# winlaic/ZipVoice

Measured on AMD Instinct MI355X. Metric: generated mel-frames/s (whole job) + RTF, ZipVoice 123M N_steps=16 batch=32/GPU, higher is better.
Workload: dtype bf16; 1 GPU; C2: ZipVoice 123M, N_steps=16, batch=32/GPU x (3 s prompt + 10 s generated; T=1219 frames), CFG g=1.0 (64 decoder rows per GPU), t_shift=0.5; model=zipvoice (zipvoice_base.json, synthetic seeded weights), global_batch=32, seq_len=1219, parallelism=dp1

## Files before the change

include/zipvoice_hip.h:

```cpp
#ifndef ZIPVOICE_HIP_H
#define ZIPVOICE_HIP_H

#include <stdint.h>

#ifdef __cplusplus
extern "C" {
#endif

typedef struct zv_engine* zv_handle;

enum zv_variant { ZV_ZIPVOICE = 0, ZV_DISTILL = 1, ZV_DIALOG = 2, ZV_DIALOG_STEREO = 3 };
enum zv_precision { ZV_FP32 = 0, ZV_BF16 = 1, ZV_MIXED = 2, ZV_FP8 = 3 };

#define ZV_MAX_STACKS 8

typedef struct {
  int variant;
  int precision;
  int feat_dim;
  int num_stacks;
  int downsampling_factor[ZV_MAX_STACKS];
  int num_layers[ZV_MAX_STACKS];
  int cnn_module_kernel[ZV_MAX_STACKS];
  int fm_decoder_dim, fm_decoder_feedforward_dim, fm_decoder_num_heads;
  int text_encoder_num_layers, text_encoder_feedforward_dim, text_encoder_cnn_module_kernel;
  int text_encoder_num_heads, text_encoder_dim;
  int time_embed_dim, text_embed_dim;
  int query_head_dim, value_head_dim, pos_head_dim, pos_dim;
  int vocab_size, pad_id, spk_a_id, spk_b_id;
} zv_config;

const char* zv_last_error(void);
const char* zv_version(void);

zv_handle zv_create(const zv_config* cfg);
void zv_destroy(zv_handle h);

int zv_set_weight(zv_handle h, const char* name, const float* host_data, int64_t numel);
int zv_finalize(zv_handle h);
int zv_reserve(zv_handle h, int max_batch, int max_frames);
int64_t zv_device_bytes(zv_handle h);

enum zv_padding { ZV_PAD_BATCH = 0, ZV_PAD_ROW = 1 };
int zv_set_padding(zv_handle h, int mode);
int zv_get_padding(zv_handle h);

int zv_profile(int enable);
int zv_profile_report(char* buf, int buflen);

int64_t zv_host_block_count(void);

int zv_attn_fallbacks(zv_handle h, int reset, int64_t* host_counts);

int zv_attn2_check(int kernel, int form, int B, int L, int H, int nv, const float* qkp, const float* P,
                   const uint8_t* key_pad, const float* v, const float* y, int force_exact, float* out,
                   int64_t* counts);

int zv_bench_gemm(int M, int N, int K, int variant, int iters, int out_mode, float* ms_out);

int zv_bench_fused_linear(int form, int M, int N, int K, int rpb, int iters, float* ms_out);

int zv_gemm_selftest(int M, int N, int K, int variant, int mode, float* maxdiff, float* maxref);

enum zv_linear_form {
  ZV_LIN_PLAIN = 0,
  ZV_LIN_PLAIN_F32 = 1,
  ZV_LIN_RESID = 2,
  ZV_LIN_RESID_BYP = 3,
  ZV_LIN_RESID_RV = 4,
  ZV_LIN_RESID_RV_COPY = 5,
  ZV_LIN_TRANS = 6,
  ZV_LIN_NA = 7,
  ZV_LIN_GLU = 8,
  ZV_LIN_GLU_DW = 9
};
typedef struct {
  int M, N, K, split, form, act;
  int rows_per_group;
  int rpb;
  int guard;
  const float* A; const float* W; const float* bias;
  const float* resid;
  const float* orig;
  const float* byp;
  const float* rowvec;
  const uint8_t* rowmask;
  const float* dw_w;
  const float* dw_b;
  int dw_ks, dw_L;
  float* C; int64_t ldc;
  uint16_t* Ch; uint16_t* Cl; int64_t ldch;
  uint16_t* Cth; uint16_t* Ctl; int64_t ldct;
  int launch[8];
  int num_cus;
} zv_linear_check_args;
int zv_linear_check(zv_linear_check_args* a);

typedef struct {
  int M, H, form, rows_per_group, part_slots, guard;
  float log_scale;
  const float* x; const float* W1; const float* b1; const float* W2; const float* b2;
  const float* resid;
  const float* rowvec;
  const float* orig;
  const float* byp;
  const float* nb;
  float* C; int64_t ldc;
  uint16_t* Ch; uint16_t* Cl; uint16_t* C2h; uint16_t* C2l; int64_t ldch;
  int launch[8];
// ... 323 lines not shown
```

zipvoice_amd/csrc/zv_checks.inc:

```
#pragma once

namespace {

struct ChkDev {
  std::vector<void*> ptrs;
  void* raw(size_t bytes) {
    void* p = nullptr;
    ZV_CHECK(ZV_BLOCKING(hipMalloc(&p, bytes + 256)));
    ptrs.push_back(p);
    return p;
  }
  template <typename T> T* make(size_t n) { return reinterpret_cast<T*>(raw(n * sizeof(T))); }
  template <typename T> T* zero(size_t n) {
    T* d = make<T>(n);
    ZV_CHECK(ZV_BLOCKING(hipMemset(d, 0, n * sizeof(T))));
    return d;
  }
  template <typename T> T* up(const T* host, size_t n) {
    T* d = make<T>(n);
    ZV_CHECK(ZV_BLOCKING(hipMemcpy(d, host, n * sizeof(T), hipMemcpyHostToDevice)));
    return d;
  }
  template <typename T> void down(T* host, const T* dev, size_t n) {
    ZV_CHECK(ZV_BLOCKING(hipMemcpy(host, dev, n * sizeof(T), hipMemcpyDeviceToHost)));
// ... 198 lines not shown
      p.Ch = reinterpret_cast<bf16*>(R) + (size_t)k * M * N;
      p.ldch = N;
    }
    if (mode == 2) {
      ZV_CHECK(hipMemcpyAsync(outs[k], R, mn * 4, hipMemcpyDeviceToDevice, s));
      p.resid = outs[k];
    }
    if (k == 0) launch_gemm<128, 128, 2, 2, 1, EPI_STD, 2, 2>(p, 1, s, "ref", true, 0);
    else if (variant == 70) launch_gemm<128, 128, 2, 2, 1, EPI_STD, 2, 2, GEMM_BK, 0, 0, 1>(p, 1, s, "t", true, -1);
    else if (variant == 71) launch_gemm<128, 128, 2, 2, 1, EPI_STD, 2, 2, GEMM_BK, 0, 0, 2>(p, 1, s, "t", true, -1);
    else launch_gemm<128, 128, 2, 2, 1, EPI_STD, 2, 2, GEMM_BK, 0, 0, 3>(p, 1, s, "t", true, -1);
  }
  if (bf16_out)
    for (int k = 0; k < 2; ++k)
      hipLaunchKernelGGL(zv_bf16_to_f32_kernel, dim3(1024), dim3(256), 0, s,
                         reinterpret_cast<bf16*>(R) + (size_t)k * M * N, outs[k], (long)M * N);
  ZV_CHECK(hipMemsetAsync(res, 0, 8, s));
  hipLaunchKernelGGL(zv_maxdiff_kernel, dim3(1024), dim3(256), 0, s, outs[1], outs[0], (long)M * N, res);
  float h[2];
  dev.down(h, res, 2);
  *maxdiff = h[0]; *maxref = h[1];
  ZV_API_END
}

int zv_attn_plan(int split, int sa_plo, int tpm, int L, int nv_na, int64_t* lds_sa, int64_t* lds_na,
                 int64_t* lds_stats, int* fits) {
  ZV_API_BEGIN
  ZV_REQUIRE((split == 1 || split == 3) && L > 0 && nv_na > 0 && sa_plo >= -1 && sa_plo <= 1 &&
                 tpm >= 0 && tpm <= 3 && (split == 1 || (sa_plo < 0 && tpm == 0)) && lds_sa && lds_na &&
                 lds_stats && fits,
             "bad arguments");
  if (tpm == 3) {
    *lds_sa = (int64_t)(sa3_qpw(L) ? sa3_plan_lds(L) : sa2_qpw(L) == 3 ? sa2_lds_bytes<3>(L) : sa2_lds_bytes<2>(L));
    *lds_na = (int64_t)(nv_na <= 128 ? na2_lds_bytes<1, 8>(L) : nv_na <= 256 ? na2_lds_bytes<2, 8>(L) : na2_lds_bytes<3, 8>(L));
    *lds_stats = 0;
    *fits = fused_attn2_fits(L, nv_na);
    return 0;
  }
  *lds_sa = (int64_t)(sa_plo < 0 ? sa_lds_bytes(L) : (sa_plo ? sa_tp_lds_bytes<1>(L) : sa_tp_lds_bytes<0>(L)));
  *lds_na = (int64_t)(split == 1 ? na_lds_bytes_for<1>(L, nv_na, tpm) : na_lds_bytes_for<3>(L, nv_na, tpm));
  *lds_stats = (int64_t)pos_mask_bytes(L, 64, true);
  *fits = split == 1 ? fused_attn_fits<1>(L, nv_na, sa_plo, tpm) : fused_attn_fits<3>(L, nv_na, sa_plo, tpm);
  ZV_API_END
}

int zv_attn2_check(int kernel, int form, int B, int L, int H, int nv, const float* qkp, const float* P,
                   const uint8_t* key_pad, const float* v, const float* y, int force_exact, float* out,
                   int64_t* counts) {
  ZV_API_BEGIN
  ZV_REQUIRE((kernel == 0 || kernel == 1) && B > 0 && L > 0 && H > 0 && qkp && P && v && out &&
                 (kernel == 0 ? (nv > 0 && nv <= 12) : (nv > 0 && nv <= 384 && y)),
             "zv_attn2_check: bad arguments");
  ZV_REQUIRE(kernel != 0 || (form >= 0 && form <= 5), "zv_attn2_check: SelfAttention form 0..5");
  ZV_REQUIRE(kernel != 1 || (form >= 0 && form <= 2), "zv_attn2_check: NonlinAttention form 0..2");
  const long ldq = 2L * H * ATT_QD + H * ATT_PD, M = (long)B * L, Lpad = round_up(L, 64);
  const long vrows = kernel == 0 ? 16L * H : nv;
  std::vector<bf16> hq((size_t)M * ldq), hv((size_t)B * vrows * Lpad, (bf16)0.f);
  for (size_t i = 0; i < hq.size(); ++i) hq[i] = (bf16)qkp[i];
  for (int b = 0; b < B; ++b)
    for (long r = 0; r < vrows; ++r) {
      const int h = kernel == 0 ? (int)(r / 16) : 0, d = kernel == 0 ? (int)(r % 16) : (int)r;
      for (int j = 0; j < L; ++j) {
        float x = 0.f;
        if (kernel == 1) x = v[((long)b * L + j) * nv + d];
        else if (d < nv) x = v[((long)b * L + j) * H * nv + (long)h * nv + d];
        else if (d == 12) x = 1.f;
        hv[((size_t)b * vrows + r) * Lpad + j] = (bf16)x;
      }
    }
  std::vector<bf16> hy;
  if (kernel == 1) {
    hy.resize((size_t)M * nv);
    for (size_t i = 0; i < hy.size(); ++i) hy[i] = (bf16)y[i];
  }
  const long ocols = kernel == 0 ? (long)H * nv : nv, ldo = round_up(ocols, 8);
  ChkDev dev;
  bf16* dout = dev.zero<bf16>((size_t)M * ldo);
  unsigned* dcnt = dev.zero<unsigned>(4);
  FlashParams f{};
  f.qh = dev.up(hq.data(), hq.size()); f.ldq = ldq;
  f.P = dev.up(P, (size_t)(2 * L - 1) * H * ATT_PD);
  f.key_pad = key_pad ? dev.up(key_pad, (size_t)M) : nullptr;
  f.B = B; f.L = L; f.H = H;
  f.vh = dev.up(hv.data(), hv.size()); f.ldv = Lpad; f.sv_b = vrows * Lpad; f.nv = nv;
  f.oh = dout; f.ldo = ldo;
  f.force_exact = force_exact; f.fallback = dcnt;
  hipStream_t s = nullptr;
  if (kernel == 0) {
    f.vrows_per_head = 16; f.ocol_per_head = nv;
    launch_attn_sa_b2(f, form ? form : sa_b2_form(L), s);
  } else {
    f.vrows_per_head = 0; f.ocol_per_head = 0;
    f.mulh = dev.up(hy.data(), hy.size()); f.ldmul = nv;
    launch_attn_na_b2(f, nv, form ? form : na_b2_form(L), s);
  }
  ZV_CHECK(ZV_BLOCKING(hipDeviceSynchronize()));
  std::vector<bf16> ho((size_t)M * ldo);
  dev.down(ho.data(), dout, ho.size());
  for (long m = 0; m < M; ++m)
    for (long c = 0; c < ocols; ++c) out[m * ocols + c] = (float)ho[m * ldo + c];
  if (counts) {
    unsigned c[4];
    dev.down(c, dcnt, 4);
    for (int i = 0; i < 3; ++i) counts[i] = c[i];
  }
  ZV_API_END
}

int zv_mx8_quantize(const float* x, int rows, int K, uint8_t* q, uint8_t* s) {
  ZV_API_BEGIN
  ZV_REQUIRE(x && q && s && rows >= 0 && K > 0, "bad arguments");
  mx8_quantize_host(x, K, rows, K, q, round_up(K, MX8_KSTEP), s);
  ZV_API_END
}

int zv_mx8_gemm_check(int M, int N, int K, const float* A, const float* W, float* C, uint8_t* Aq,
                      uint8_t* As) {
  ZV_API_BEGIN
  ZV_REQUIRE(A && W && C && M > 0 && N > 0 && K > 0 && K % MX8_KSTEP == 0 && N % 8 == 0,
             "zv_mx8_gemm_check: K a multiple of 128, N of 8");
  hipStream_t s = nullptr;
  const long Np = round_up(N, 128);
  std::vector<bf16> ah((size_t)M * K);
  for (size_t i = 0; i < ah.size(); ++i) ah[i] = (bf16)A[i];
  std::vector<float> wp((size_t)Np * K, 0.f);
  memcpy(wp.data(), W, (size_t)N * K * 4);
  std::vector<uint8_t> wq((size_t)Np * K), ws((size_t)Np * K / MX8_BLOCK);
  mx8_quantize_host(wp.data(), K, (int)Np, K, wq.data(), K, ws.data());
  ChkDev dev;
  uint8_t* dAq = dev.make<uint8_t>((size_t)M * K);
  uint8_t* dAs = dev.make<uint8_t>((size_t)M * K / MX8_BLOCK);
  const uint8_t* dWq = dev.up(wq.data(), wq.size());
  const uint8_t* dWs = dev.up(ws.data(), ws.size());
  float* dC = dev.zero<float>((size_t)M * N);
  Act a16;
  a16.h = dev.up(ah.data(), ah.size()); a16.ld = K;
  a16.q = dAq; a16.qs = dAs; a16.ldq = K;
  LinearPolicy().pack8(a16, M, K, s);
  GemmParams p{};
  p.M = M; p.N = N; p.K = K; p.nz2 = 1; p.Brows = (int)Np;
  p.Ah = reinterpret_cast<const bf16*>(dAq); p.lda = K; p.As = dAs; p.ldas = K / MX8_BLOCK;
  p.Bh = reinterpret_cast<const bf16*>(dWq); p.ldb = K; p.Bs = dWs; p.ldbs = K / MX8_BLOCK;
  p.bias = dev.zero<float>((size_t)N); p.C = dC; p.ldc = N; p.resid = dC; p.rows_per_group = 1; p.rpb = 1;
  launch_gemm<128, 128, 2, 2, 8, EPI_STD, 2, 2, MX8_KSTEP, 0, 0, 1>(p, 1, s, "mx8_check", true, -1);
  ZV_CHECK(ZV_BLOCKING(hipDeviceSynchronize()));
  dev.down(C, dC, (size_t)M * N);
  if (Aq) dev.down(Aq, dAq, (size_t)M * K);
  if (As) dev.down(As, dAs, (size_t)M * K / MX8_BLOCK);
  ZV_API_END
}

int zv_linear_check(zv_linear_check_args* a) {
  ZV_API_BEGIN
  ZV_REQUIRE(a && a->M > 0 && a->N > 0 && a->K > 0 && a->A && a->W && a->bias && a->guard >= 0 &&
                 (a->split == 1 || a->split == 2 || a->split == 3) && a->form >= ZV_LIN_PLAIN &&
                 a->form <= ZV_LIN_GLU_DW,
             "zv_linear_check: bad arguments");
  const int M = a->M, N = a->N, K = a->K, form = a->form, G = a->guard;
// ... 1107 lines not shown
```

zipvoice_amd/csrc/zv_engine.hip:

```cpp
#include <math.h>
#include <stdlib.h>
#include <string.h>

#include <algorithm>
#include <map>
#include <memory>
#include <mutex>
#include <string>
#include <exception>
#include <functional>
#include <tuple>
#include <vector>


#include "zv_common.h"
#include "zv_gemm.inc"
#include "zv_gemm256.inc"
#include "zv_ffn.inc"
#include "zv_attn.inc"
#include "zv_elem.inc"
#include "zv_session.inc"
#include "zv_flash.inc"
#include "zv_flash2.inc"
#include "zv_weights.inc"
// ... 131 lines not shown
  StreamSet set;
  set.dev = dev;
  for (int i = 0; i < ZV_STREAM_SET; ++i)
    ZV_CHECK(ZV_BLOCKING(hipStreamCreateWithFlags(&set.s[i], hipStreamNonBlocking)));
  return set;
}
static void release_stream_set(const StreamSet& set) {
  if (set.dev < 0) return;
  for (hipStream_t st : set.s)
    if (st) (void)ZV_BLOCKING(hipStreamSynchronize(st));
  std::lock_guard<std::mutex> lock(g_stream_pool_mu);
  stream_pool_free().push_back(set);
}

}

struct zv_engine;
struct zv_session {
  zv_engine* eng = nullptr;
  int slots = 0, maxT = 0;
  DBuf x, tc, sc, pad;
  float *dx = nullptr, *dtc = nullptr, *dsc = nullptr;
  uint8_t* dpad = nullptr;
  std::vector<SchedRow> rows;
  std::vector<std::vector<float>> ts;
  std::vector<int> lens, done;
  int64_t ticks = 0, dec_rows = 0, dec_row_frames = 0, last_T = 0;
  ~zv_session();
};

struct zv_engine : LinearPolicy {
  zv_config cfg;
  WeightStore store;
  ZipformerW dec, txt;
  float* embed_table = nullptr;
  float* spk_table = nullptr;
  float* temb_freqs = nullptr;
  Workspace ws_dec, ws_txt;
  static constexpr int MAX_SPLIT = 4;
  Workspace ws_split[MAX_SPLIT - 1];
  int split_streams = 3;
  long split_min_rows = 0;
  hipStream_t split_stream[MAX_SPLIT - 1] = {};
  hipEvent_t split_fork = nullptr, split_join[MAX_SPLIT - 1] = {};

  bool materialize_attn = false;
  int ffn_fused = 3;
  long ffn_min_rows = 15000;
  int fp8_fuse = 7;
  int sa_tp = 1;
  bool mixed_sa = true;
  bool attn_b2 = false, attn_b2_dec = false;
  int attn2_exact = 0;
  int glu_dw = 1;
  unsigned* attn_fallback = nullptr;
  int padding = ZV_PAD_BATCH;

  explicit zv_engine(const zv_config& c) : cfg(c) {
    auto envi = [](const char* k, int d) { const char* v = getenv(k); return v ? atoi(v) : d; };
    materialize_attn = envi("ZV_ATTN_MATERIALIZE", 0) == 1;
    graph_mode = envi("ZV_GRAPH", 2);
    sa_tp = envi("ZV_SA_TP", 1);
    fp8_fuse = envi("ZV_FP8_FUSE", 7);
    ffn_fused = envi("ZV_FFN", 3);
    ffn_min_rows = envi("ZV_FFN_MIN_ROWS", 15000);
    ffn_persist = envi("ZV_FFN_PERSIST", 1);
    split_streams = envi("ZV_SPLIT_STREAMS", 3);
    split_min_rows = envi("ZV_SPLIT_MIN_ROWS", 8192);
    mixed_sa = envi("ZV_MIXED_SA", 1) != 0;
    attn_b2 = envi("ZV_ATTN2", 1) != 0 && (cfg.precision == ZV_BF16 || cfg.precision == ZV_FP8);
    attn_b2_dec = attn_b2 || (envi("ZV_ATTN2", 1) != 0 && cfg.precision == ZV_MIXED);
    attn2_exact = envi("ZV_ATTN2_EXACT", 0) != 0;
    glu_dw = envi("ZV_GLU_DW", 1);
  }
  struct GraphKey {
    int B, T, N, has_pad;
    float g, t0, t1, shift;
    int cfg_mode;
    int padding;
    unsigned long gen;
    bool operator<(const GraphKey& o) const {
      return std::tie(B, T, N, has_pad, g, t0, t1, shift, cfg_mode, padding, gen) <
             std::tie(o.B, o.T, o.N, o.has_pad, o.g, o.t0, o.t1, o.shift, o.cfg_mode, o.padding, o.gen);
    }
  };
  static constexpr size_t MAX_GRAPHS = 8, MAX_SEEN = 256;
  struct GraphEntry { hipGraphExec_t exec; unsigned long last_use; };
  std::map<GraphKey, GraphEntry> graphs;
  std::map<GraphKey, int> graph_seen;
  unsigned long graph_clock = 0;
  hipStream_t gstream = nullptr;
  hipEvent_t gev_in = nullptr, gev_out = nullptr;
  DBuf gx, gtc, gsc, gpad, ggrows;
  int graph_mode = 2;

  int ffn_persist = 1;
  void attach_ffn_scratch(FfnParams& q, Workspace& ws) {
    if (!ffn_persist) return;
    const int cus = zv_num_cus();
    q.part = ws.ffn_part.get<float>((size_t)cus * FFN_PART_FLOATS);
    unsigned* fl = ws.ffn_flag.get<unsigned>((size_t)cus + 64);
    q.flag = fl;
    q.part_slots = cus;
  }
  void ffn_site(FfnParams q, Workspace& ws, hipStream_t s, const char* tag) {
    attach_ffn_scratch(q, ws);
    launch_ffn(q, s, tag);
  }

  void check_dev_err() {
    volatile unsigned* e = zv_dev_err_host();
    if (*e == 0) return;
    ZV_CHECK(ZV_BLOCKING(hipDeviceSynchronize()));
    auto clear = [](Workspace& w) {
      if (w.ffn_flag.p) ZV_CHECK(ZV_BLOCKING(hipMemset(w.ffn_flag.p, 0, w.ffn_flag.bytes)));
    };
    clear(ws_dec); clear(ws_txt);
    for (Workspace& w : ws_split) clear(w);
    ZV_CHECK(ZV_BLOCKING(hipDeviceSynchronize()));
    *e = 0;
    throw std::runtime_error("fused FeedForward: a C item waited more than 2 s for its producer's tiles; "
                             "the outputs of the calls since the previous one are invalid (schedule flags reset)");
  }

  void drop_graphs() {
// ... 274 lines not shown
                    false, attn_b2);
    embed_table = store.upload_key("embed.weight", (size_t)cfg.vocab_size * cfg.text_embed_dim);
    if (dialog()) spk_table = store.upload_key("spk_embed.weight", (size_t)2 * F);
    const int half = cfg.time_embed_dim / 2;
    std::vector<float> fr(half);
    for (int k = 0; k < half; ++k)
      fr[k] = expf((float)(-log(10000.0)) * (float)k / (float)half);
    temb_freqs = store.dalloc<float>(half);
    ZV_CHECK(ZV_BLOCKING(hipMemcpy(temb_freqs, fr.data(), half * sizeof(float), hipMemcpyHostToDevice)));
    attn_fallback = store.dalloc<unsigned>(4);
    ZV_CHECK(ZV_BLOCKING(hipMemset(attn_fallback, 0, 4 * sizeof(unsigned))));
    size_t expected = count_expected();
    if (expected != store.staged.size())
      throw std::invalid_argument("state dict has " + std::to_string(store.staged.size()) +
                                  " tensors, config expects " + std::to_string(expected) +
                                  " (unexpected keys present)");
    store.staged.clear();
    store.derived.clear();
    store.ready = true;
  }

  size_t count_expected() const {
    auto zf = [&](const ZipformerW& Z) {
      size_t n = 4 * Z.in_proj.size();
      for (const auto& S : Z.stacks) {
        if (S.ds != 1) n += 2;
        if (Z.temb_dim > 0) n += 2;
        n += S.layers.size() * 43;
      }
      if (Z.has_time) n += 4;
      if (Z.has_guid) n += 1;
      return n;
    };
    return zf(dec) + zf(txt) + 1 + (dialog() ? 1 : 0);
  }

  void small_linear(const Linear& L, const float* in, int ldin, int M, float* out, int ldout,
                    int pre, const float* add, hipStream_t s) {
    launch_small_linear(in, ldin, L.w32, L.K, L.b, add, out, ldout, M, L.N, L.K, pre, -1, s);
  }

  bool fp8_mode() const { return cfg.precision == ZV_FP8; }

  template <int SPLIT, int TPM>
  static void attn_na_v1(const FlashParams& f, int hid, hipStream_t s) {
    constexpr int QTILES = SPLIT == 3 ? 4 : 8;
    if (hid <= 128) launch_attn_na<SPLIT, 1, QTILES, TPM>(f, s);
    else if (hid <= 256) launch_attn_na<SPLIT, 2, QTILES, TPM>(f, s);
    else launch_attn_na<SPLIT, 3, QTILES, TPM>(f, s);
  }
  template <int SPLIT>
  void attn_na(const FlashParams& f, int hid, bool a2, bool tp_na, hipStream_t s) {
    if constexpr (SPLIT == 1) {
      if (a2) return launch_attn_na_b2(f, hid, na_b2_form(f.L), s);
      if (tp_na) return attn_na_v1<1, 1>(f, hid, s);
    }
    attn_na_v1<SPLIT, 0>(f, hid, s);
  }
  template <int SPLIT>
  void attn_sa(const FlashParams& f, bool a2, hipStream_t s) {
    if constexpr (SPLIT == 1) {
      if (a2) return launch_attn_sa_b2(f, sa_b2_form(f.L), s);
      if (sa_tp) {
        if (sa_tp == 3) launch_attn_sa_tp<0, 1>(f, s);
        else launch_attn_sa_tp<0>(f, s);
        return;
      }
    }
    launch_attn_sa<SPLIT>(f, s);
  }

  template <int SPLIT>
  void layer(const Pass& pass, const ZipformerW& Z, const LayerW& W, Workspace& ws, float* src,
             Act src_a, float* cur, Act cur_a, int B, int L, const uint8_t* pad, const float* posP,
             const float* temb, bool has_next, hipStream_t s, bool fresh8 = false) {
    const bool split = SPLIT == 3;
    const long M = (long)B * L;
    const long Mtot = pass.batch_rows > 0 ? pass.batch_rows * (long)L : M;
    const int D = Z.dim, H = Z.heads;
    const long Lpad = round_up(L, 64);
    const char* tag_att = split ? "gemm_attn_fp32" : "gemm_attn_bf16";
    const int qkpN = W.attn_in.N;
    Act qkp = ws.qkp.get(M, qkpN, split);
    {
      Out o; o.act = qkp;
      if (SPLIT == 1 && pass.io_split) attn_in_wsplit(W.attn_in, src_a, M, o, s);
      else linear<SPLIT>(W.attn_in, src_a, M, o, s);
    }
    const bool tp_na = SPLIT == 1 && sa_tp;
    const int sa_plo = (SPLIT == 1 && sa_tp) ? 0 : -1;
    const bool a2 = SPLIT == 1 && Z.b2;
    const bool materialize = materialize_attn || (a2 ? !fused_attn2_fits(L, W.na_in.N / 3)
                                                     : !fused_attn_fits<SPLIT>(L, W.na_in.N / 3, sa_plo, tp_na ? 1 : 0));
    Act Wt;
    FlashParams fp{};
    if (materialize) {
      Wt = ws.W.get((long)H * M, Lpad, split);
      AttnParams ap{qkp.h, qkp.l, qkpN, posP, pad, Wt.h, Wt.l, Lpad, B, L, H, a2 ? 1 : 0};
      launch_attn_softmax<SPLIT>(ap, s);
    } else {
      fp.qh = qkp.h; fp.ql = qkp.l; fp.ldq = qkpN; fp.P = posP; fp.key_pad = pad;
      fp.B = B; fp.L = L; fp.H = H;
      fp.force_exact = attn2_exact; fp.fallback = attn_fallback;
      if (!a2) {
        fp.stats = ws.stats.get<float2>((size_t)M);
        if constexpr (SPLIT == 1)
          if (tp_na) launch_attn_stats<1, 1>(fp, s);
// ... 1347 lines not shown
```

zipvoice_amd/csrc/zv_flash2.inc:

```
#pragma once
#include "zv_flash.inc"

constexpr float FA2_MASKED = -1000.f * 1.4426950408889634f;
constexpr float FA2_DEN_LO = 8.673617379884035e-19f;
constexpr float FA2_DEN_HI = 1.2676506002282294e30f;
constexpr int SA2_KS = 64;
constexpr bool FA2_OFS = std::is_same<bf16, _Float16>::value;
#ifndef ZV_FA2_DIAG
#define ZV_FA2_DIAG 1
#endif

template <int KS>
__device__ __forceinline__ void stage_bias2(const FlashParams& p, int b, float* Mb, uint8_t* Fs, int tid,
                                            int nt) {
  const int L = p.L, nks = (L + KS - 1) / KS, NM = nks * KS;
  for (int k = tid; k < nks; k += nt) Fs[k] = 0;
  __syncthreads();
  const uint8_t* kp = p.key_pad ? p.key_pad + (long)b * L : nullptr;
  for (int t = tid; t < NM; t += nt) {
    const int m = t >= L ? 2 : (kp ? kp[t] : 0);
    Mb[t] = m == 0 ? 0.f : (m == 1 ? FA2_MASKED : -INFINITY);
    if (m) Fs[t / KS] = 1;
  }
  __syncthreads();
// ... 519 lines not shown
      c = ZV_MFMA_16x16x32(ldk(ks * FA_KB), qf, c, 0, 0, 0);
      c = ZV_MFMA_16x16x32(PP[jb + tbl], pb[0], c, 0, 0, 0);
      c = ZV_MFMA_16x16x32(PP[jb + tbl - 8], pb[1], c, 0, 0, 0);
      mx = fmaxf(mx, fmaxf(fmaxf(c[0], c[1]), fmaxf(c[2], c[3])));
    }
    half_sums(mx, true);
    const float rowmax = ceilf(fmaxf(Qs[sq * 16 + c16], Qs[QT + sq * 16 + c16]));
    cofs = f32x4{0.f, 0.f, 0.f, 0.f};
    __syncthreads();
    key_loop(rowmax);
    half_sums(psum, false);
  }

#pragma unroll
  for (int q = 0; q < 4; ++q) {
    const int ql = (aq0 + q) * 16 + c16;
    const int qo = qt0 + ql;
    if (qo >= L) continue;
    const float rden = 1.f / (Qs[ql] + Qs[QT + ql]);
    const long orow = (long)b * L + qo;
#pragma unroll
    for (int t = 0; t < DTW; ++t) {
      const int d0 = (ad0 + t) * 16 + g * 4;
      if (d0 >= nv) continue;
      float v[4] = {acc[q][t][0], acc[q][t][1], acc[q][t][2], acc[q][t][3]};
      float y[4];
      load_split4(p.mulh, (const bf16*)nullptr, orow * p.ldmul + d0, y);
#pragma unroll
      for (int e = 0; e < 4; ++e) v[e] *= y[e] * rden;
      store_split4(p.oh, nullptr, orow * p.ldo + d0, v);
    }
  }
}

inline int na2_qtiles(int L) { return L <= 900 ? 4 : 8; }

template <int DTW, int QTILES = 8>
static void launch_attn_na2(const FlashParams& p, hipStream_t s) {
  const size_t lds = na2_lds_bytes<DTW, QTILES>(p.L);
  ZV_REQUIRE(lds <= 160 * 1024, "sequence too long for the fused attention kernel");
  ZV_REQUIRE(p.nv <= 8 * DTW * 16 && !p.ol && p.ldq % 8 == 0, "NonlinAttention v2 operands");
  static unsigned long long attr = 0;
  if (!((attr >> zv_cur_device()) & 1)) {
    ZV_CHECK(hipFuncSetAttribute((const void*)zv_attn_na2_kernel<DTW, QTILES>,
                                 hipFuncAttributeMaxDynamicSharedMemorySize, 160 * 1024));
    attr |= 1ull << zv_cur_device();
  }
  const long nblk = (long)cdiv(p.L, 16 * QTILES) * p.B;
  ZvProfScope prof("attn_na_bf16", (72.0 + 2.0 * p.nv) * p.B * (double)p.L * p.L, 0.0, s);
  hipLaunchKernelGGL((zv_attn_na2_kernel<DTW, QTILES>), dim3((unsigned)nblk), dim3(128 * QTILES), lds, s, p);
  ZV_LAUNCH_CHECK();
}

constexpr int SA3_SLOT = 6144;
template <int QPW>
__host__ __device__ inline size_t sa3_lds_bytes(int L) {
  const int nks = (L + SA2_KS - 1) / SA2_KS;
  return (size_t)3 * SA3_SLOT + (size_t)(L + 64 * QPW + SA2_KS) * 16 + (size_t)nks * SA2_KS * 4 + round_up(nks, 16);
}

inline int sa3_qpw(int L) {
  if (L <= 400) return 0;
  if (L >= 1500 && sa3_lds_bytes<3>(L) <= 80 * 1024) return 3;
  if (L >= 1000 && L < 1500 && sa3_lds_bytes<4>(L) <= 80 * 1024) return 4;
  return sa3_lds_bytes<2>(L) <= 80 * 1024 ? 2 : 0;
}
inline int sa2_qpw(int L) { return L > 400 && sa2_lds_bytes<3>(L) <= 160 * 1024 ? 3 : 2; }
inline size_t sa3_plan_lds(int L) {
  const int q = sa3_qpw(L);
  return q == 4 ? sa3_lds_bytes<4>(L) : q == 3 ? sa3_lds_bytes<3>(L) : q == 2 ? sa3_lds_bytes<2>(L) : 0;
}

template <int QPW, int MINW = 2>
__global__ __launch_bounds__(256, MINW) void zv_attn_sa3_kernel(FlashParams p) {
  constexpr int QT = 64 * QPW, KS = SA2_KS, NU = QPW + 3;
  extern __shared__ __attribute__((aligned(16))) unsigned char fsm[];
  const int L = p.L;
  const int nks = (L + KS - 1) / KS;
  const int NT = L + QT + KS;
  unsigned char* ring = fsm;
  bf16x8* PP = reinterpret_cast<bf16x8*>(fsm + 3 * SA3_SLOT);
  float* Mb = reinterpret_cast<float*>(PP + NT);
  uint8_t* Fs = reinterpret_cast<uint8_t*>(Mb + nks * KS);

  const int nqb = (L + QT - 1) / QT;
  const int lb = fa2_xcd_block(blockIdx.x, gridDim.x);
  const int qt0 = (lb % nqb) * QT, h = (lb / nqb) % p.H, b = lb / nqb / p.H;
  const int tid = threadIdx.x, lane = tid & 63;
  const int wave = __builtin_amdgcn_readfirstlane(tid >> 6);
  const int g = lane >> 4, c16 = lane & 15;
  const long qbase = (long)b * L * p.ldq;

  const int ldqb = (int)p.ldq * 2, ldvb = (int)p.ldv * 2;
  const char* kbase = reinterpret_cast<const char*>(p.qh + qbase + p.H * ATT_QD + h * ATT_QD);
  const char* vbase = reinterpret_cast<const char*>(p.vh + (long)b * p.sv_b + (long)h * 16 * p.ldv);
  const unsigned k_lane = (unsigned)(c16 * ldqb + g * 16);
  const int vrow = 8 * (wave & 1) + (lane >> 3);
  const unsigned v_lane = (unsigned)(vrow * ldvb + (((lane & 7) ^ ((vrow >> 1) & 7)) * 16));
  auto issue = [&](int ks) {
    unsigned char* slot = ring + (ks % 3) * SA3_SLOT;
    const int j0 = ks * KS, jk = j0 + 16 * wave;
    if (jk + 16 <= L) {
      glds16s(kbase + (long)jk * ldqb, k_lane, slot + wave * 1024);
    } else {
      const unsigned kc = (unsigned)(min(jk + c16, L - 1) * ldqb + g * 16);
      glds16s(kbase, kc, slot + wave * 1024);
// ... 188 lines not shown
  }

#pragma unroll
  for (int qq = 0; qq < QPW; ++qq) {
    const int d0 = g * 4;
    if (qi[qq] >= L || d0 >= p.nv) continue;
    const float rden = 1.f / den[qq];
    float v[4] = {acc[qq][0] * rden, acc[qq][1] * rden, acc[qq][2] * rden, acc[qq][3] * rden};
    const long o = ((long)b * L + qi[qq]) * p.ldo + (long)h * p.ocol_per_head + d0;
    if (d0 + 3 < p.nv) {
      store_split4(p.oh, p.ol, o, v);
      if (p.oh2) store_split4(p.oh2, nullptr, o, v);
    } else {
      for (int e = 0; d0 + e < p.nv; ++e) {
        split_store(p.oh, p.ol, o + e, v[e]);
        if (p.oh2) split_store(p.oh2, nullptr, o + e, v[e]);
      }
    }
  }
}

template <int QPW = 2, int MINW = 2>
static void launch_attn_sa3(const FlashParams& p, hipStream_t s) {
  const size_t lds = sa3_lds_bytes<QPW>(p.L);
  ZV_REQUIRE(lds <= 160 * 1024, "sequence too long for the fused attention kernel");
  ZV_REQUIRE(p.nv <= 12 && p.vrows_per_head == 16 && p.ldq % 8 == 0 && p.ldv % 64 == 0,
             "SelfAttention v3: 16-row value heads (row 12 = ones), V^T rows padded to 64 keys");
  static unsigned long long attr = 0;
  if (!((attr >> zv_cur_device()) & 1)) {
    ZV_CHECK(hipFuncSetAttribute((const void*)zv_attn_sa3_kernel<QPW, MINW>,
                                 hipFuncAttributeMaxDynamicSharedMemorySize, 160 * 1024));
    attr |= 1ull << zv_cur_device();
  }
  const long nblk = (long)cdiv(p.L, 64 * QPW) * p.H * p.B;
  ZV_REQUIRE(nblk < (1L << 31), "SelfAttention v3 grid");
  ZvProfScope prof("attn_sa_bf16", (72.0 + 2.0 * p.nv) * p.H * p.B * (double)p.L * p.L, 0.0, s);
  hipLaunchKernelGGL((zv_attn_sa3_kernel<QPW, MINW>), dim3((unsigned)nblk), dim3(256), lds, s, p);
  ZV_LAUNCH_CHECK();
}

inline int sa_b2_form(int L) {
  const int q3 = sa3_qpw(L);
  return q3 ? q3 + 1 : sa2_qpw(L) == 3 ? 2 : 1;
}
static void launch_attn_sa_b2(const FlashParams& f, int form, hipStream_t s) {
  switch (form) {
    case 1: launch_attn_sa2<2>(f, s); break;
    case 2: launch_attn_sa2<3, 1>(f, s); break;
    case 3: launch_attn_sa3<2>(f, s); break;
    case 4: launch_attn_sa3<3>(f, s); break;
    default: launch_attn_sa3<4>(f, s); break;
  }
}
inline int na_b2_form(int L) { return na2_qtiles(L) == 4 ? 1 : 2; }
static void launch_attn_na_b2(const FlashParams& f, int hid, int form, hipStream_t s) {
  if (hid <= 128) { if (form == 1) launch_attn_na2<1, 4>(f, s); else launch_attn_na2<1>(f, s); }
  else if (hid <= 256) { if (form == 1) launch_attn_na2<2, 4>(f, s); else launch_attn_na2<2>(f, s); }
  else if (form == 1) launch_attn_na2<3, 4>(f, s);
  else launch_attn_na2<3>(f, s);
}

static bool fused_attn2_fits(int L, int nv_na) {
  const size_t lim = 160 * 1024;
  const size_t na = nv_na <= 128 ? na2_lds_bytes<1, 8>(L) : nv_na <= 256 ? na2_lds_bytes<2, 8>(L) : na2_lds_bytes<3, 8>(L);
  return sa2_lds_bytes<2>(L) <= lim && na <= lim;
}
```

zipvoice_amd/engine.py:

```python
from __future__ import annotations

import ctypes
import os
from typing import Dict, Optional

import numpy as np
import torch

from .config import ModelConfig
from .weights import check_state_dict

LIB_NAME = "libzipvoice_hip.so"
LIB_PATH = os.path.join(os.path.dirname(os.path.abspath(__file__)), LIB_NAME)
LIB_F16_PATH = os.path.join(os.path.dirname(os.path.abspath(__file__)), "libzipvoice_hip_f16.so")
MAX_STACKS = 8
VARIANT_ID = {"zipvoice": 0, "zipvoice_distill": 1, "zipvoice_dialog": 2,
              "zipvoice_dialog_stereo": 3}
PRECISION_ID = {"fp32": 0, "bf16": 1}
MODES = {"fp32": ("bf16", 0), "bf16": ("bf16", 1), "fp16": ("f16", 2),
         "fp16_plain": ("f16", 1), "bf16_mixed": ("bf16", 2), "fp8": ("bf16", 3)}


class ZvConfig(ctypes.Structure):
    _fields_ = [
# ... 116 lines not shown

def row_schedule_array(schedule):
    arr = (ZvRowSched * len(schedule))()
    for i, r in enumerate(schedule):
        if isinstance(r, (tuple, list)):
            n, t0, t1, sh, g = r
        else:
            n, t0, t1, sh, g = r.num_step, r.t_start, r.t_end, r.t_shift, r.guidance_scale
        if int(n) != n:
            raise ValueError(f"schedule row {i}: num_step must be an integer, got {n!r}")
        arr[i] = ZvRowSched(int(n), float(t0), float(t1), float(sh), float(g))
    return arr


class ZvNoiseCheckArgs(ctypes.Structure):
    _fields_ = [("mode", ctypes.c_int), ("where", ctypes.c_int),
                ("counter", ctypes.c_uint32 * 4), ("key", ctypes.c_uint32 * 2),
                ("count", ctypes.c_int64),
                ("words", ctypes.c_void_p), ("bits", ctypes.c_void_p), ("normals", ctypes.c_void_p)]


_P = ctypes.c_void_p
_I = ctypes.c_int
_F = ctypes.c_float
SIGNATURES = {
    "zv_last_error": (ctypes.c_char_p, []),
    "zv_version": (ctypes.c_char_p, []),
    "zv_create": (_P, [ctypes.POINTER(ZvConfig)]),
    "zv_destroy": (None, [_P]),
    "zv_set_weight": (_I, [_P, ctypes.c_char_p, _P, ctypes.c_int64]),
    "zv_finalize": (_I, [_P]),
    "zv_reserve": (_I, [_P, _I, _I]),
    "zv_device_bytes": (ctypes.c_int64, [_P]),
    "zv_set_padding": (_I, [_P, _I]),
    "zv_get_padding": (_I, [_P]),
    "zv_profile": (_I, [_I]),
    "zv_bench_gemm": (_I, [_I, _I, _I, _I, _I, _I, ctypes.POINTER(ctypes.c_float)]),
    "zv_bench_fused_linear": (_I, [_I, _I, _I, _I, _I, _I, ctypes.POINTER(ctypes.c_float)]),
    "zv_gemm_selftest": (_I, [_I, _I, _I, _I, _I, ctypes.POINTER(ctypes.c_float), ctypes.POINTER(ctypes.c_float)]),
    "zv_linear_check": (_I, [ctypes.POINTER(ZvLinearCheckArgs)]),
    "zv_ffn_check": (_I, [ctypes.POINTER(ZvFfnCheckArgs)]),
    "zv_dwconv_check": (_I, [ctypes.POINTER(ZvDwconvCheckArgs)]),
    "zv_stackedge_check": (_I, [ctypes.POINTER(ZvStackedgeCheckArgs)]),
    "zv_padrow_check": (_I, [ctypes.POINTER(ZvPadrowCheckArgs)]),
    "zv_bigvgan_check": (_I, [ctypes.POINTER(ZvBigvganCheckArgs)]),
    "zv_solve_check": (_I, [ctypes.POINTER(ZvSolveCheckArgs)]),
    "zv_time_steps": (_I, [_F, _F, _I, _F, _P]),
    "zv_cfg_plan": (_I, [_F, _F, _I, _I, _I, _P, _P, _P, _P]),
    "zv_profile_report": (_I, [ctypes.c_char_p, _I]),
    "zv_host_block_count": (ctypes.c_int64, []),
    "zv_attn_fallbacks": (_I, [_P, _I, _P]),
    "zv_attn2_check": (_I, [_I, _I, _I, _I, _I, _I, _P, _P, _P, _P, _P, _I, _P, _P]),
    "zv_attn_plan": (_I, [_I, _I, _I, _I, _I, _P, _P, _P, _P]),
    "zv_mx8_quantize": (_I, [_P, _I, _I, _P, _P]),
    "zv_mx8_gemm_check": (_I, [_I, _I, _I, _P, _P, _P, _P, _P]),
    "zv_fm_decoder": (_I, [_P, _P, _P, _P, _P, _P, _P, _I, _I, _I, _P, _P]),
    "zv_velocity": (_I, [_P, _F, _F, _P, _P, _P, _P, _I, _I, _P, _P]),
    "zv_euler_sample": (_I, [_P, _P, _P, _P, _P, _I, _I, _I, _F, _F, _F, _F, _P]),
    "zv_velocity_rows": (_I, [_P, _F, _P, _P, _P, _P, _P, _I, _I, _P, _P]),
    "zv_euler_sample_rows": (_I, [_P, _P, _P, _P, _P, _I, _I, _I, _P, _F, _F, _F, _P]),
    "zv_euler_sample_sched": (_I, [_P, _P, _P, _P, _P, _I, _I, _P, _P]),
    "zv_sched_stats": (_I, [_P, _P]),
    "zv_sched_plan": (_I, [_P, _I, _I, _I, ctypes.POINTER(ZvSchedPlanOut)]),
    "zv_sched_check": (_I, [ctypes.POINTER(ZvSchedCheckArgs)]),
    "zv_session_create": (_P, [_P, _I, _I]),
    "zv_session_destroy": (None, [_P]),
    "zv_session_admit": (_I, [_P, _I, _P, _P, _P, _P, _P, _P, _I, _P]),
    "zv_session_step": (_I, [_P, _P]),
    "zv_session_retire": (_I, [_P, _I, _P, _P, _I, _P]),
    "zv_session_state": (_I, [_P, _P, _P]),
    "zv_session_plan": (_I, [_P, _P, _P, _I, _I, ctypes.POINTER(ZvSchedPlanOut), _P]),
    "zv_session_check": (_I, [ctypes.POINTER(ZvSessionCheckArgs)]),
    "zv_text_encode": (_I, [_P, _P, _P, _P, _I, _I, _P, _P]),
    "zv_text_condition": (_I, [_P, _P, _I, _I, _P, _P, _I, _P, _P]),
    "zv_speech_condition": (_I, [_P, _P, _I, _I, _I, _P, _I, _P, _P]),
    "zv_vocoder_create": (_P, [_P]),
    "zv_vocoder_destroy": (None, [_P]),
    "zv_vocoder_set_weight": (_I, [_P, ctypes.c_char_p, _P, ctypes.c_int64]),
    "zv_vocoder_finalize": (_I, [_P]),
    "zv_vocoder_decode": (_I, [_P, _P, _I, _F, _F, _P, _I, _I, _P, _I, _P]),
    "zv_vocoder_device_bytes": (ctypes.c_int64, [_P]),
    "zv_bigvgan_create": (_P, [_P]),
    "zv_bigvgan_destroy": (None, [_P]),
    "zv_bigvgan_set_weight": (_I, [_P, ctypes.c_char_p, _P, ctypes.c_int64]),
    "zv_bigvgan_finalize": (_I, [_P]),
    "zv_bigvgan_decode": (_I, [_P, _P, _I, _F, _F, _P, _I, _I, _P, _P]),
    "zv_bigvgan_device_bytes": (ctypes.c_int64, [_P]),
    "zv_fbank_create": (_P, [_I, _I, _I, _P, _P]),
    "zv_fbank_destroy": (None, [_P]),
    "zv_fbank_extract": (_I, [_P, _P, ctypes.c_int64, _P, _I, _I, _P, ctypes.c_int64, _P]),
    "zv_fbank_configure": (_I, [_P, _I, _F, _F]),
    "zv_resample_create": (_P, [_I, _I, _I, _P, _P]),
    "zv_resample_destroy": (None, [_P]),
    "zv_resample_apply": (_I, [_P, _P, ctypes.c_int64, _P, _I, _P, ctypes.c_int64, ctypes.c_int64, _P]),
    "zv_resample_device_bytes": (ctypes.c_int64, [_P]),
    "zv_wavjoin_create": (_P, [_I, _F, _I, _I, _I]),
    "zv_wavjoin_destroy": (None, [_P]),
    "zv_wavjoin_apply": (_I, [_P, _P, ctypes.c_int64, _P, _P, _I, _I, _P, ctypes.c_int64,
                              ctypes.c_int64, _P, _P, _P]),
    "zv_wavjoin_apply_docs": (_I, [_P, _P, ctypes.c_int64, _P, _P, _I, _I, _P, _I, _P,
                                   ctypes.c_int64, ctypes.c_int64, _P, _P, _P]),
    "zv_wavjoin_device_bytes": (ctypes.c_int64, [_P]),
    "zv_wavjoin_stream_create": (_P, [_P, _I, _I]),
    "zv_wavjoin_stream_destroy": (None, [_P]),
    "zv_wavjoin_stream_reset": (_I, [_P, _I, _P]),
    "zv_wavjoin_stream_push": (_I, [_P, _P, ctypes.c_int64, _P, _P, _I, _P, _P, _P, ctypes.c_int64,
# ... 479 lines not shown
```

Measured before the change: 87690 mel-frames/s.

## Add third-generation NonlinAttention kernel with double-buffered V and software-pipelined scores

Adds a new NonlinAttention kernel (na3) that double-buffers V tiles and score probabilities in LDS. It prefetches K fragments ahead and interleaves score computation for the next key block with the MFMA accumulation of the current one. The engine selects it by default whenever the LDS plan fits under 160 KiB, with ZV_ATTN3=0 as an opt-out. The aim is to hide global-load and exp latency in the attention path, at the cost of larger LDS use and possibly lower occupancy.

```diff
diff --git a/include/zipvoice_hip.h b/include/zipvoice_hip.h
--- a/include/zipvoice_hip.h
+++ b/include/zipvoice_hip.h
@@ -55,6 +55,8 @@
 int zv_attn2_check(int kernel, int form, int B, int L, int H, int nv, const float* qkp, const float* P,
                    const uint8_t* key_pad, const float* v, const float* y, int force_exact, float* out,
                    int64_t* counts);
+
+int zv_attn3_plan(int form, int L, int nv, int64_t* lds, int* engine_form);
 
 int zv_bench_gemm(int M, int N, int K, int variant, int iters, int out_mode, float* ms_out);
 
diff --git a/zipvoice_amd/csrc/zv_checks.inc b/zipvoice_amd/csrc/zv_checks.inc
--- a/zipvoice_amd/csrc/zv_checks.inc
+++ b/zipvoice_amd/csrc/zv_checks.inc
@@ -274,7 +274,7 @@
                  (kernel == 0 ? (nv > 0 && nv <= 12) : (nv > 0 && nv <= 384 && y)),
              "zv_attn2_check: bad arguments");
   ZV_REQUIRE(kernel != 0 || (form >= 0 && form <= 5), "zv_attn2_check: SelfAttention form 0..5");
-  ZV_REQUIRE(kernel != 1 || (form >= 0 && form <= 2), "zv_attn2_check: NonlinAttention form 0..2");
+  ZV_REQUIRE(kernel != 1 || (form >= 0 && form <= 4), "zv_attn2_check: NonlinAttention form 0..4");
   const long ldq = 2L * H * ATT_QD + H * ATT_PD, M = (long)B * L, Lpad = round_up(L, 64);
   const long vrows = kernel == 0 ? 16L * H : nv;
   std::vector<bf16> hq((size_t)M * ldq), hv((size_t)B * vrows * Lpad, (bf16)0.f);
@@ -314,7 +314,8 @@
   } else {
     f.vrows_per_head = 0; f.ocol_per_head = 0;
     f.mulh = dev.up(hy.data(), hy.size()); f.ldmul = nv;
-    launch_attn_na_b2(f, nv, form ? form : na_b2_form(L), s);
+    const char* e3 = getenv("ZV_ATTN3");
+    launch_attn_na_b2(f, nv, form ? form : na_b2_form(L, nv, !e3 || atoi(e3) != 0), s);
   }
   ZV_CHECK(ZV_BLOCKING(hipDeviceSynchronize()));
   std::vector<bf16> ho((size_t)M * ldo);
@@ -326,6 +327,14 @@
     dev.down(c, dcnt, 4);
     for (int i = 0; i < 3; ++i) counts[i] = c[i];
   }
+  ZV_API_END
+}
+
+int zv_attn3_plan(int form, int L, int nv, int64_t* lds, int* engine_form) {
+  ZV_API_BEGIN
+  ZV_REQUIRE((form == 3 || form == 4) && L > 0 && nv > 0 && nv <= 384 && lds && engine_form, "bad arguments");
+  *lds = (int64_t)na3_plan_lds(L, nv, form == 3 ? 4 : 8);
+  *engine_form = na_b2_form(L, nv, true);
   ZV_API_END
 }
 
diff --git a/zipvoice_amd/csrc/zv_engine.hip b/zipvoice_amd/csrc/zv_engine.hip
--- a/zipvoice_amd/csrc/zv_engine.hip
+++ b/zipvoice_amd/csrc/zv_engine.hip
@@ -207,6 +207,7 @@
   bool mixed_sa = true;
   bool attn_b2 = false, attn_b2_dec = false;
   int attn2_exact = 0;
+  bool attn3 = true;
   int glu_dw = 1;
   unsigned* attn_fallback = nullptr;
   int padding = ZV_PAD_BATCH;
@@ -226,6 +227,7 @@
     attn_b2 = envi("ZV_ATTN2", 1) != 0 && (cfg.precision == ZV_BF16 || cfg.precision == ZV_FP8);
     attn_b2_dec = attn_b2 || (envi("ZV_ATTN2", 1) != 0 && cfg.precision == ZV_MIXED);
     attn2_exact = envi("ZV_ATTN2_EXACT", 0) != 0;
+    attn3 = envi("ZV_ATTN3", 1) != 0;
     glu_dw = envi("ZV_GLU_DW", 1);
   }
   struct GraphKey {
@@ -606,7 +608,7 @@
   template <int SPLIT>
   void attn_na(const FlashParams& f, int hid, bool a2, bool tp_na, hipStream_t s) {
     if constexpr (SPLIT == 1) {
-      if (a2) return launch_attn_na_b2(f, hid, na_b2_form(f.L), s);
+      if (a2) return launch_attn_na_b2(f, hid, na_b2_form(f.L, hid, attn3), s);
       if (tp_na) return attn_na_v1<1, 1>(f, hid, s);
     }
     attn_na_v1<SPLIT, 0>(f, hid, s);
diff --git a/zipvoice_amd/csrc/zv_flash2.inc b/zipvoice_amd/csrc/zv_flash2.inc
--- a/zipvoice_amd/csrc/zv_flash2.inc
+++ b/zipvoice_amd/csrc/zv_flash2.inc
@@ -595,6 +595,265 @@
   ZV_LAUNCH_CHECK();
 }
 
+constexpr int NA3_KS = 64;
+template <int DTW, int QTILES>
+__host__ __device__ inline size_t na3_lds_bytes(int L) {
+  const int nkb = (L + NA3_KS - 1) / NA3_KS;
+  return (size_t)2 * (8 * DTW * 16) * 128 +
+         (size_t)2 * (2 * QTILES) * 1024 +
+         (size_t)(L + QTILES * 16 + NA3_KS) * 16 +
+         (size_t)nkb * NA3_KS * 4 +
+         round_up(nkb, 16) +
+         (size_t)2 * QTILES * 16 * 4 + 16;
+}
+
+template <int DTW, int QTILES, int ABL = 0>
+__global__ __launch_bounds__(128 * QTILES) void zv_attn_na3_kernel(FlashParams p) {
+  constexpr int NT = 128 * QTILES, NW = 2 * QTILES, KS = NA3_KS;
+  constexpr int QT = 16 * QTILES;
+  constexpr int NTILE = 8 * DTW;
+  constexpr int VSLOT = NTILE * 16 * 128;
+  constexpr int PPW = 2 * NTILE / NW;
+  constexpr int PSET = 2 * QTILES * 1024;
+  static_assert(QTILES % 4 == 0, "4 query tiles per accumulating wave");
+  static_assert((2 * NTILE) % NW == 0, "whole pieces per wave");
+  extern __shared__ __attribute__((aligned(16))) unsigned char fsm[];
+  const int L = p.L;
+  const int nkb = (L + KS - 1) / KS;
+  const int NTB = L + QT + KS;
+  unsigned char* Vs = fsm;
+  unsigned char* Pf = Vs + 2 * VSLOT;
+  bf16x8* PP = reinterpret_cast<bf16x8*>(Pf + 2 * PSET);
+  float* Mb = reinterpret_cast<float*>(PP + NTB);
+  uint8_t* Fs = reinterpret_cast<uint8_t*>(Mb + nkb * KS);
+  float* Qs = reinterpret_cast<float*>(Fs + round_up(nkb, 16));
+  int* bflag = reinterpret_cast<int*>(Qs + 2 * QT);
+
+  const int nqb = (L + QT - 1) / QT;
+  const int lb = fa2_xcd_block(blockIdx.x, gridDim.x);
+  const int qt0 = (lb % nqb) * QT, b = lb / nqb;
+  const int tid = threadIdx.x, lane = tid & 63;
+  const int wave = __builtin_amdgcn_readfirstlane(tid >> 6);
+  const int g = lane >> 4, c16 = lane & 15;
+  const long qbase = (long)b * L * p.ldq;
+
+  const int sq = wave >> 1, hh = wave & 1;
+  const int qi = qt0 + sq * 16 + c16;
+  const int qc = min(qi, L - 1);
+  const int kperm = 8 * (c16 >> 2) + (c16 & 3);
+  bf16x8 qf, pb[2];
+  int tbl = 0;
+  if (tid == 0) *bflag = 0;
+  stage_tp<0>(p, 0, qt0, QT, NTB, PP, nullptr, tid, NT);
+  stage_bias2<KS>(p, b, Mb, Fs, tid, NT);
+  tp_query(p, qbase + (long)qc * p.ldq, 0, c16, g, qt0 + sq * 16, qt0, QT, qf, pb, tbl);
+  tbl += hh * 32 + kperm - c16;
+  const int ldqb = (int)p.ldq * 2;
+  const __amdgpu_buffer_rsrc_t rsK = __builtin_amdgcn_make_buffer_rsrc(
+      const_cast<bf16*>(p.qh + qbase + p.H * ATT_QD), 0, (L - 1) * ldqb + 2 * ATT_QD, 0x00020000);
+  const int vk = (hh * 32 + kperm) * ldqb + g * 16;
+  struct KF { decltype(__builtin_amdgcn_raw_buffer_load_b128(rsK, 0, 0, 0)) t[2]; };
+  auto ldk = [&](int ks) -> KF {
+    const int o = vk + ks * KS * ldqb;
+    KF k;
+    k.t[0] = __builtin_amdgcn_raw_buffer_load_b128(rsK, o, 0, 0);
+    k.t[1] = __builtin_amdgcn_raw_buffer_load_b128(rsK, o + 4 * ldqb, 0, 0);
+    return k;
+  };
+  const int aq0 = (wave >> 3) * 4, ad0 = (wave & 7) * DTW;
+  const int ldvb = (int)p.ldv * 2;
+  const char* vbase = reinterpret_cast<const char*>(p.vh + (long)b * p.sv_b);
+  unsigned voff[PPW];
+#pragma unroll
+  for (int c = 0; c < PPW; ++c) {
+    const int pc = wave + c * NW, r16 = (pc & 1) * 8 + (lane >> 3);
+    voff[c] = (unsigned)(min((pc >> 1) * 16 + r16, p.nv - 1) * ldvb + (((lane & 7) ^ ((r16 >> 1) & 7)) * 16));
+  }
+  auto issue = [&](int ks) {
+    unsigned char* slot = Vs + (ks & 1) * VSLOT;
+    const char* src = vbase + (long)ks * KS * 2;
+#pragma unroll
+    for (int c = 0; c < PPW; ++c) glds16s(src, voff[c], slot + (wave + c * NW) * 1024);
+  };
+  auto wait_step = [&](KF& k) {
+    if constexpr (ABL == 5) asm volatile("s_waitcnt vmcnt(0) lgkmcnt(0)" : "+v"(k.t[0]), "+v"(k.t[1])::"memory");
+    else asm volatile("s_waitcnt vmcnt(0) lgkmcnt(0)\n\ts_barrier" : "+v"(k.t[0]), "+v"(k.t[1])::"memory");
+  };
+
+  f32x4 acc[4][DTW];
+  float psum = 0.f;
+  f32x4 cofs = {0.f, 0.f, 0.f, 0.f};
+  auto score_raw = [&](auto BIAS_, int ks, const KF& kf, f32x4 (&c)[2]) {
+    const int jb = ks * KS;
+#pragma unroll
+    for (int u = 0; u < 2; ++u) {
+      if constexpr (decltype(BIAS_)::value)
+        c[u] = *reinterpret_cast<const f32x4*>(Mb + jb + hh * 32 + g * 8 + u * 4) + cofs;
+      else c[u] = cofs;
+    }
+#pragma unroll
+    for (int u = 0; u < 2; ++u) {
+      c[u] = ZV_MFMA_16x16x32(__builtin_bit_cast(bf16x8, kf.t[u]), qf, c[u], 0, 0, 0);
+      c[u] = ZV_MFMA_16x16x32(PP[jb + tbl + 4 * u], pb[0], c[u], 0, 0, 0);
+      c[u] = ZV_MFMA_16x16x32(PP[jb + tbl + 4 * u - 8], pb[1], c[u], 0, 0, 0);
+    }
+  };
+  auto score_step = [&](int ks, const KF& kf, float sub) {
+    f32x4 c[2];
+    if (__builtin_amdgcn_readfirstlane(Fs[ks])) score_raw(std::true_type{}, ks, kf, c);
+    else score_raw(std::false_type{}, ks, kf, c);
+    bf16x8 ph;
+#pragma unroll
+    for (int e = 0; e < 8; ++e) {
+      const float pr = __builtin_amdgcn_exp2f(c[e >> 2][e & 3] - sub);
+      psum += pr;
+      ph[e] = (bf16)pr;
+    }
+    *reinterpret_cast<bf16x8*>(Pf + (ks & 1) * PSET + ((hh * QTILES + sq) * 64 + lane) * 16) = ph;
+  };
+  const int vsw = (c16 >> 1) & 7;
+  auto accumulate_step = [&](int ks, int s2a, int s2b) {
+    const unsigned char* vb = Vs + (ks & 1) * VSLOT;
+    const unsigned char* pbuf = Pf + (ks & 1) * PSET;
+#pragma unroll
+    for (int s2 = s2a; s2 < s2b; ++s2) {
+      bf16x8 va[DTW];
+#pragma unroll
+      for (int t = 0; t < DTW; ++t)
+        va[t] = *reinterpret_cast<const bf16x8*>(vb + ((ad0 + t) * 16 + c16) * 128 + (((s2 * 4 + g) ^ vsw) * 16));
+#pragma unroll
+      for (int q = 0; q < 4; ++q) {
+        const bf16x8 pbh = *reinterpret_cast<const bf16x8*>(pbuf + ((s2 * QTILES + aq0 + q) * 64 + lane) * 16);
+#pragma unroll
+        for (int t = 0; t < DTW; ++t) acc[q][t] = ZV_MFMA_16x16x32(va[t], pbh, acc[q][t], 0, 0, 0);
+      }
+    }
+  };
+  auto key_loop = [&](float sub) {
+#pragma unroll
+    for (int q = 0; q < 4; ++q)
+#pragma unroll
+      for (int t = 0; t < DTW; ++t) acc[q][t] = f32x4{0.f, 0.f, 0.f, 0.f};
+    psum = 0.f;
+    KF kf = ldk(0);
+    issue(0);
+    score_step(0, kf, sub);
+    if (nkb > 1) kf = ldk(1);
+    for (int kb = 0; kb < nkb; ++kb) {
+      wait_step(kf);
+      if (kb + 1 < nkb && ABL != 1) issue(kb + 1);
+      if (ABL != 4) accumulate_step(kb, 0, 1);
+      if (kb + 1 < nkb) {
+        if (ABL != 3) score_step(kb + 1, kf, sub);
+        if (kb + 2 < nkb && ABL != 2) kf = ldk(kb + 2);
+      }
+      if (ABL != 4) accumulate_step(kb, 1, 2);
+    }
+  };
+  auto half_sums = [&](float x, bool is_max) {
+#pragma unroll
+    for (int o = 16; o <= 32; o <<= 1) {
+      const float y = __shfl_xor(x, o, 64);
+      x = is_max ? fmaxf(x, y) : x + y;
+    }
+    if (g == 0) Qs[hh * QT + sq * 16 + c16] = x;
+    __syncthreads();
+  };
+  auto max8 = [](const f32x4 (&c)[2]) {
+    return fmaxf(fmaxf(fmaxf(c[0][0], c[0][1]), fmaxf(c[0][2], c[0][3])),
+                 fmaxf(fmaxf(c[1][0], c[1][1]), fmaxf(c[1][2], c[1][3])));
+  };
+
+  if constexpr (FA2_OFS) {
+    const int ksd = fa2_diag_step<KS>(Mb, min((qt0 + sq * 16) / KS, nkb - 1), lane);
+    float ml = -1e30f;
+#pragma unroll
+    for (int e = 0; e < (ZV_FA2_DIAG ? 2 : 1); ++e) {
+      f32x4 c[2];
+      score_raw(std::true_type{}, e ? ksd : 0, ldk(e ? ksd : 0), c);
+      ml = fmaxf(ml, max8(c));
+    }
+    half_sums(ml, true);
+    const float off = ceilf(fmaxf(Qs[sq * 16 + c16], Qs[QT + sq * 16 + c16]));
+    cofs = f32x4{-off, -off, -off, -off};
+  }
+  key_loop(0.f);
+  half_sums(psum, false);
+  if (tid < QT) {
+    const float den = Qs[tid] + Qs[QT + tid];
+    if (qt0 + tid < L) {
+      if (den < FA2_DEN_LO) atomicOr(bflag, 1);
+      if (!(den <= FA2_DEN_HI)) atomicOr(bflag, 2);
+    }
+  }
+  __syncthreads();
+  bool nonfinite = false;
+#pragma unroll
+  for (int q = 0; q < 4; ++q)
+#pragma unroll
+    for (int t = 0; t < DTW; ++t)
+#pragma unroll
+      for (int r = 0; r < 4; ++r) nonfinite |= !(fabsf(acc[q][t][r]) <= 3.4e38f);
+  if (__builtin_amdgcn_ballot_w64(nonfinite) != 0 && lane == 0) atomicOr(bflag, 2);
+  __syncthreads();
+  const int bf = *bflag;
+  if (bf || p.force_exact) {
+    if (tid == 0) fa2_count(p, bf & 1, bf & 2);
+    cofs = f32x4{0.f, 0.f, 0.f, 0.f};
+    float mx = -1e30f;
+    for (int ks = 0; ks < nkb; ++ks) {
+      f32x4 c[2];
+      score_raw(std::true_type{}, ks, ldk(ks), c);
+      mx = fmaxf(mx, max8(c));
+    }
+    half_sums(mx, true);
+    const float rowmax = ceilf(fmaxf(Qs[sq * 16 + c16], Qs[QT + sq * 16 + c16]));
+    __syncthreads();
+    key_loop(rowmax);
+    half_sums(psum, false);
+  }
+
+  const int nv = p.nv;
+#pragma unroll
+  for (int q = 0; q < 4; ++q) {
+    const int ql = (aq0 + q) * 16 + c16;
+    const int qo = qt0 + ql;
+    if (qo >= L) continue;
+    const float rden = 1.f / (Qs[ql] + Qs[QT + ql]);
+    const long orow = (long)b * L + qo;
+#pragma unroll
+    for (int t = 0; t < DTW; ++t) {
+      const int d0 = (ad0 + t) * 16 + g * 4;
+      if (d0 >= nv) continue;
+      float v[4] = {acc[q][t][0], acc[q][t][1], acc[q][t][2], acc[q][t][3]};
+      float y[4];
+      load_split4(p.mulh, (const bf16*)nullptr, orow * p.ldmul + d0, y);
+#pragma unroll
+      for (int e = 0; e < 4; ++e) v[e] *= y[e] * rden;
+      store_split4(p.oh, nullptr, orow * p.ldo + d0, v);
+    }
+  }
+}
+
+template <int DTW, int QTILES = 8, int ABL = 0>
+static void launch_attn_na3(const FlashParams& p, hipStream_t s) {
+  const size_t lds = na3_lds_bytes<DTW, QTILES>(p.L);
+  ZV_REQUIRE(lds <= 160 * 1024, "sequence too long for the third-generation NonlinAttention kernel");
+  ZV_REQUIRE(p.nv <= 8 * DTW * 16 && !p.ol && p.ldq % 8 == 0 && p.ldv % 8 == 0 && p.sv_b % 8 == 0 &&
+                 p.ldv >= round_up(p.L, NA3_KS),
+             "NonlinAttention v3 operands: V^T rows padded to 64 keys");
+  static unsigned long long attr = 0;
+  if (!((attr >> zv_cur_device()) & 1)) {
+    ZV_CHECK(hipFuncSetAttribute((const void*)zv_attn_na3_kernel<DTW, QTILES, ABL>,
+                                 hipFuncAttributeMaxDynamicSharedMemorySize, 160 * 1024));
+    attr |= 1ull << zv_cur_device();
+  }
+  const long nblk = (long)cdiv(p.L, 16 * QTILES) * p.B;
+  ZvProfScope prof("attn_na_bf16", (72.0 + 2.0 * p.nv) * p.B * (double)p.L * p.L, 0.0, s);
+  hipLaunchKernelGGL((zv_attn_na3_kernel<DTW, QTILES, ABL>), dim3((unsigned)nblk), dim3(128 * QTILES), lds, s, p);
+  ZV_LAUNCH_CHECK();
+}
+
 constexpr int SA3_SLOT = 6144;
 template <int QPW>
 __host__ __device__ inline size_t sa3_lds_bytes(int L) {
@@ -889,12 +1148,29 @@
     default: launch_attn_sa3<4>(f, s); break;
   }
 }
-inline int na_b2_form(int L) { return na2_qtiles(L) == 4 ? 1 : 2; }
+inline size_t na3_plan_lds(int L, int hid, int qtiles) {
+  if (qtiles == 4)
+    return hid <= 128 ? na3_lds_bytes<1, 4>(L) : hid <= 256 ? na3_lds_bytes<2, 4>(L) : na3_lds_bytes<3, 4>(L);
+  return hid <= 128 ? na3_lds_bytes<1, 8>(L) : hid <= 256 ? na3_lds_bytes<2, 8>(L) : na3_lds_bytes<3, 8>(L);
+}
+inline int na_b2_form(int L, int hid, bool gen3) {
+  const int qt = na2_qtiles(L);
+  const int f = qt == 4 ? 1 : 2;
+  return gen3 && na3_plan_lds(L, hid, qt) <= 160 * 1024 ? f + 2 : f;
+}
+template <int DTW>
+static void launch_attn_na_b2_w(const FlashParams& f, int form, hipStream_t s) {
+  switch (form) {
+    case 1: launch_attn_na2<DTW, 4>(f, s); break;
+    case 2: launch_attn_na2<DTW, 8>(f, s); break;
+    case 3: launch_attn_na3<DTW, 4>(f, s); break;
+    default: launch_attn_na3<DTW, 8>(f, s); break;
+  }
+}
 static void launch_attn_na_b2(const FlashParams& f, int hid, int form, hipStream_t s) {
-  if (hid <= 128) { if (form == 1) launch_attn_na2<1, 4>(f, s); else launch_attn_na2<1>(f, s); }
-  else if (hid <= 256) { if (form == 1) launch_attn_na2<2, 4>(f, s); else launch_attn_na2<2>(f, s); }
-  else if (form == 1) launch_attn_na2<3, 4>(f, s);
-  else launch_attn_na2<3>(f, s);
+  if (hid <= 128) launch_attn_na_b2_w<1>(f, form, s);
+  else if (hid <= 256) launch_attn_na_b2_w<2>(f, form, s);
+  else launch_attn_na_b2_w<3>(f, form, s);
 }
 
 static bool fused_attn2_fits(int L, int nv_na) {
diff --git a/zipvoice_amd/engine.py b/zipvoice_amd/engine.py
--- a/zipvoice_amd/engine.py
+++ b/zipvoice_amd/engine.py
@@ -192,6 +192,7 @@
     "zv_attn_fallbacks": (_I, [_P, _I, _P]),
     "zv_attn2_check": (_I, [_I, _I, _I, _I, _I, _I, _P, _P, _P, _P, _P, _I, _P, _P]),
     "zv_attn_plan": (_I, [_I, _I, _I, _I, _I, _P, _P, _P, _P]),
+    "zv_attn3_plan": (_I, [_I, _I, _I, _P, _P]),
     "zv_mx8_quantize": (_I, [_P, _I, _I, _P, _P]),
     "zv_mx8_gemm_check": (_I, [_I, _I, _I, _P, _P, _P, _P, _P]),
     "zv_fm_decoder": (_I, [_P, _P, _P, _P, _P, _P, _P, _I, _I, _I, _P, _P]),
```

Result: no change. 88340 mel-frames/s (median of 6 runs) (+0.7%).
